# p2004dr/visual-slam

Measured on AMD Instinct MI355X. Metric: frames/sec (extract+match+pose) at 640×480, 2000 ORB, 1/2/4/8 MI355X, higher is better.
Workload: dtype u8

## Files before the change

visual-slam_amd/csrc/orb_kernels.hip:

```cpp
#include <cstring>

#include "common.h"
#include "select_replay.h"
#include "fast_score.h"

__constant__ __attribute__((aligned(16))) int8_t c_pattern[256 * 4] = {
#include "orb_pattern.inc"
};

#define WAVE 64

__device__ __forceinline__ int reflect101(int p, int len) {
    if (len == 1) return 0;
    while (p < 0 || p >= len) p = p < 0 ? -p : 2 * len - 2 - p;
    return p;
}

__device__ __forceinline__ void xcd_map(uint32_t lin, uint32_t per, uint32_t inv_per, uint32_t batch, int& frame, int& item) {
    const uint32_t b8 = batch & ~7u, cut = per * b8;
    const bool head = lin < cut;
    const uint32_t n = head ? lin >> 3 : lin - cut;
    const uint32_t q = inv_per ? __umulhi(n, inv_per) : n;
    item = (int)(n - q * per);
    frame = (int)(head ? (lin & 7u) + 8u * q : b8 + q);
// ... 66 lines not shown

#define RS_TW 64
#define RS_TH 64
#define RS_SRC_ROWS 136
#define RS_SRC_PITCH 144

__global__ __launch_bounds__(256) void k_resize(const uint8_t* __restrict__ src, size_t src_fstride, int spitch, int sw, int sh,
                                                uint8_t* __restrict__ dst, size_t dst_fstride, int dpitch, int dw, int dh,
                                                const int* __restrict__ xofs, const int* __restrict__ xc1,
                                                const int* __restrict__ yofs, const int* __restrict__ yc1,
                                                uint32_t inv_per, uint32_t inv_gx, int org) {
    __shared__ __attribute__((aligned(16))) uint8_t s_src[RS_SRC_ROWS * RS_SRC_PITCH];
    __shared__ int s_xo[RS_TW], s_xc[RS_TW], s_yo[RS_TH], s_yc[RS_TH];
    const int tid = threadIdx.x;
    int bx = blockIdx.x, by = blockIdx.y, bz = blockIdx.z;
    {
        int rem;
        xcd_map(bx + gridDim.x * (by + gridDim.y * bz), gridDim.x * gridDim.y, inv_per, gridDim.z, bz, rem);
        by = (int)(inv_gx ? __umulhi((uint32_t)rem, inv_gx) : (uint32_t)rem);
        bx = rem - by * (int)gridDim.x;
    }
    const int tx0 = org + bx * RS_TW, ty0 = org + by * RS_TH;
    const uint8_t* s = src + (size_t)bz * src_fstride;
    const int sx0 = xofs[tx0], sx1 = min(xofs[min(tx0 + RS_TW - 1, dw - 1)] + 1, sw - 1);
    const int sy0 = yofs[ty0], sy1 = min(yofs[min(ty0 + RS_TH - 1, dh - 1)] + 1, sh - 1);
    const int sxa = sx0 & ~3;
    const int ncols = sx1 - sxa + 1, nrows = sy1 - sy0 + 1;
    if (ncols > RS_SRC_PITCH || nrows > RS_SRC_ROWS) return;
    if (tid < RS_TW) {
        int x = min(tx0 + tid, dw - 1);
        s_xo[tid] = xofs[x];
        s_xc[tid] = xc1[x];
    } else if (tid < RS_TW + RS_TH) {
        int y = min(ty0 + tid - RS_TW, dh - 1);
        s_yo[tid - RS_TW] = yofs[y];
        s_yc[tid - RS_TW] = yc1[y];
    }
    if ((spitch & 3) == 0 && (((size_t)s) & 3) == 0) {
        const int ndw = (ncols + 3) >> 2;
        const uint32_t inv = 0x100000u / (uint32_t)ndw + 1u;
        const uint8_t* s0 = s + (size_t)sy0 * spitch + sxa;
        for (int i = tid; i < nrows * ndw; i += 256) {
            const uint32_t r = ((uint32_t)i * inv) >> 20, c4 = (uint32_t)i - r * (uint32_t)ndw;
            ((uint32_t*)(s_src + r * RS_SRC_PITCH))[c4] = *(const uint32_t*)(s0 + r * (uint32_t)spitch + 4u * c4);
        }
    } else {
        for (int i = tid; i < nrows * ncols; i += 256) {
            int r = i / ncols, cc = i - r * ncols;
            s_src[r * RS_SRC_PITCH + cc] = s[(size_t)(sy0 + r) * spitch + sxa + cc];
        }
    }
    __syncthreads();
    const int c0 = (tid & 15) * 4, x = tx0 + c0;
    if (x >= dw) return;
    int ox[4], ox1[4];
    uint32_t mx1[4];
#pragma unroll
    for (int k = 0; k < 4; k++) {
        ox[k] = s_xo[c0 + k] - sxa;
        ox1[k] = min(s_xo[c0 + k] + 1, sw - 1) - sxa;
        mx1[k] = s_xc[c0 + k];
    }
#pragma unroll
    for (int half = 0; half < RS_TH / 16; half++) {
        const int ry = (tid >> 4) + 16 * half, y = ty0 + ry;
        if (y >= dh) break;
        const int oy = s_yo[ry] - sy0, oy1 = min(s_yo[ry] + 1, sh - 1) - sy0;
        const uint32_t my1 = s_yc[ry], my0 = 256 - my1;
        const uint8_t* r0 = s_src + oy * RS_SRC_PITCH;
        const uint8_t* r1 = s_src + oy1 * RS_SRC_PITCH;
        uint32_t packed = 0;
#pragma unroll
        for (int k = 0; k < 4; k++) {
            const uint32_t mx0 = 256 - mx1[k];
            uint32_t h0 = mx0 * r0[ox[k]] + mx1[k] * r0[ox1[k]];
            uint32_t h1 = mx0 * r1[ox[k]] + mx1[k] * r1[ox1[k]];
            uint32_t v = my0 * h0 + my1 * h1;
            packed |= ((v + 32768u) >> 16) << (8 * k);
        }
        *(uint32_t*)(dst + (size_t)bz * dst_fstride + (size_t)y * dpitch + x) = packed;
    }
}


#define RS2_ROWS 136
#define RS2_UNR 5

__device__ __forceinline__ uint2 rs2_hrow(uint32_t w0, uint32_t w1, uint32_t w2, uint32_t sh8, const uint32_t (&sel)[4],
                                          const uint32_t (&coef)[4]) {
    const uint32_t u0 = __builtin_amdgcn_alignbyte(w1, w0, sh8), u1 = __builtin_amdgcn_alignbyte(w2, w1, sh8);
    uint32_t hv[4];
#pragma unroll
    for (int k = 0; k < 4; k++) hv[k] = udot2(__builtin_amdgcn_perm(u1, u0, sel[k]), coef[k], 0u);
    return make_uint2(hv[0] | (hv[1] << 16), hv[2] | (hv[3] << 16));
}

__device__ __forceinline__ uint32_t rs2_vrow(uint2 a, uint2 b, uint32_t e) {
    const uint32_t c1 = e >> 16, cy = (256u - c1) | (c1 << 16);
    const uint32_t v0 = udot2(__builtin_amdgcn_perm(b.x, a.x, 0x05040100u), cy, 32768u);
    const uint32_t v1 = udot2(__builtin_amdgcn_perm(b.x, a.x, 0x07060302u), cy, 32768u);
    const uint32_t v2 = udot2(__builtin_amdgcn_perm(b.y, a.y, 0x05040100u), cy, 32768u);
    const uint32_t v3 = udot2(__builtin_amdgcn_perm(b.y, a.y, 0x07060302u), cy, 32768u);
    return __builtin_amdgcn_perm(v1, v0, 0x0C0C0602u) | (__builtin_amdgcn_perm(v3, v2, 0x0C0C0602u) << 16);
}

__device__ __forceinline__ uint32_t hi16_pair_sat_u8(uint32_t a, uint32_t b) {
    uint32_t d;
    asm("v_sat_pk_u8_i16 %0, %1" : "=v"(d) : "v"(__builtin_amdgcn_perm(b, a, 0x07060302u)));
    return d;
}

__device__ __forceinline__ uint4 blur_row_quad(const uint32_t* pw0, const uint32_t* pw1, uint32_t g0, uint32_t g1, uint32_t g2,
                                               uint32_t g3) {
    const uint32_t ta = g0 | (g1 << 8) | (g2 << 16) | (g3 << 24), tb = g2 | (g1 << 8) | (g0 << 16);
    uint32_t o[2][4];
#pragma unroll
    for (int h = 0; h < 2; h++) {
        const uint32_t* pw = h ? pw1 : pw0;
        const uint32_t w0 = pw[0], w1 = pw[1], w2 = pw[2];
        o[h][0] = __builtin_amdgcn_udot4(__builtin_amdgcn_alignbyte(w1, w0, 1), ta, __builtin_amdgcn_udot4(__builtin_amdgcn_alignbyte(w2, w1, 1), tb, 0, false), false);
        o[h][1] = __builtin_amdgcn_udot4(__builtin_amdgcn_alignbyte(w1, w0, 2), ta, __builtin_amdgcn_udot4(__builtin_amdgcn_alignbyte(w2, w1, 2), tb, 0, false), false);
        o[h][2] = __builtin_amdgcn_udot4(__builtin_amdgcn_alignbyte(w1, w0, 3), ta, __builtin_amdgcn_udot4(__builtin_amdgcn_alignbyte(w2, w1, 3), tb, 0, false), false);
        o[h][3] = __builtin_amdgcn_udot4(w1, ta, __builtin_amdgcn_udot4(w2, tb, 0, false), false);
    }
    return make_uint4(o[0][0] | (o[1][0] << 16), o[0][1] | (o[1][1] << 16), o[0][2] | (o[1][2] << 16), o[0][3] | (o[1][3] << 16));
}

__device__ __forceinline__ void blur_col_quad(const uint32_t* sr, int pitch, uint32_t g0, uint32_t g1, uint32_t g2, uint32_t g3,
                                              uint32_t& pe, uint32_t& po) {
    const uint32_t e0 = g0 | (g1 << 16), e1 = g2 | (g3 << 16), e2 = g2 | (g1 << 16), e3 = g0;
    const uint32_t d0 = g0 << 16, d1 = g1 | (g2 << 16), d2 = g3 | (g2 << 16), d3 = g1 | (g0 << 16);
    uint4 v[4];
#pragma unroll
    for (int j = 0; j < 4; j++) v[j] = *(const uint4*)(sr + j * pitch);
    uint32_t se[4], so[4];
#pragma unroll
    for (int k = 0; k < 4; k++) {
        const uint32_t a0 = k == 0 ? v[0].x : k == 1 ? v[0].y : k == 2 ? v[0].z : v[0].w;
        const uint32_t a1 = k == 0 ? v[1].x : k == 1 ? v[1].y : k == 2 ? v[1].z : v[1].w;
        const uint32_t a2 = k == 0 ? v[2].x : k == 1 ? v[2].y : k == 2 ? v[2].z : v[2].w;
        const uint32_t a3 = k == 0 ? v[3].x : k == 1 ? v[3].y : k == 2 ? v[3].z : v[3].w;
        se[k] = udot2(a0, e0, udot2(a1, e1, udot2(a2, e2, udot2(a3, e3, 1u << 15))));
        so[k] = udot2(a0, d0, udot2(a1, d1, udot2(a2, d2, udot2(a3, d3, 1u << 15))));
    }
    pe = hi16_pair_sat_u8(se[0], se[1]) | (hi16_pair_sat_u8(se[2], se[3]) << 16);
    po = hi16_pair_sat_u8(so[0], so[1]) | (hi16_pair_sat_u8(so[2], so[3]) << 16);
}

#define RB_PW 80
#define RB_PH 80
#define RB_WR 88
#define RB_WP 96
#define RB_SR_BYTES ((RB_PH / 2 + 4) * RB_PW * 4)
struct BlurOut {
    uint8_t* dst;
    size_t fstride;
    int pitch, margin;
    uint32_t taps;
};

template <bool RS2_BLUR>
__global__ __launch_bounds__(256) void k_resize2(const uint8_t* __restrict__ src, size_t src_fstride, int spitch, int sw, int sh,
                                                 uint8_t* __restrict__ dst, size_t dst_fstride, int dpitch, int dw, int dh,
                                                 const uint32_t* __restrict__ xpk, const uint32_t* __restrict__ ypk,
                                                 uint32_t inv_per, uint32_t inv_gx, int org, BlurOut bo) {
    const int tid = threadIdx.x;
    if constexpr (RS2_BLUR) {
        __shared__ __attribute__((aligned(16))) uint8_t s_px[RB_WR * RB_WP];
        __shared__ __attribute__((aligned(16))) uint32_t s_row[RB_SR_BYTES / 4];
        int bx = blockIdx.x, by = blockIdx.y, bz = blockIdx.z;
        {
            int rem;
            xcd_map(bx + gridDim.x * (by + gridDim.y * bz), gridDim.x * gridDim.y, inv_per, gridDim.z, bz, rem);
            by = (int)(inv_gx ? __umulhi((uint32_t)rem, inv_gx) : (uint32_t)rem);
            bx = rem - by * (int)gridDim.x;
        }
        const int tx0 = org + bx * RS_TW, ty0 = org + by * RS_TH;
        const uint32_t ey0 = ypk[ty0], ey1 = ypk[ty0 + RS_TH - 1], ex1 = xpk[tx0 + RS_TW - 1];
        const int sy0 = (int)(ey0 & 0x7FFFu), sy1 = (int)(ey1 & 0x7FFFu) + (int)((ey1 >> 15) & 1u);
        const int ab0 = (int)(xpk[tx0] & 0x7FFCu), ax1 = (int)(ex1 & 0x7FFFu) + (int)((ex1 >> 15) & 1u) + 1;
        const int bm = bo.margin;
        const int r0 = by == 0 ? bm : sy0, r1 = by == (int)gridDim.y - 1 ? sh - bm : (int)(ypk[ty0 + RS_TH] & 0x7FFFu);
        const int c0 = bx == 0 ? bm : ab0, c1 = bx == (int)gridDim.x - 1 ? (sw - bm + 3) & ~3 : (int)(xpk[tx0 + RS_TW] & 0x7FFCu);
        const int wy0 = min(r0 - 3, sy0), wy1 = max(r1 + 3, sy1 + 1);
        const int wx0 = min(c0 - 4, ab0), wx1 = max(c1 + 4, (ax1 + 3) & ~3);
        const int nwr = wy1 - wy0, ndw = (wx1 - wx0) >> 2;
        const uint8_t* img = src + (size_t)bz * src_fstride;
        const int cg = tid & 15, rr = tid >> 4;
        const uint4 xe = *(const uint4*)(xpk + tx0 + 4 * cg);
        uint32_t ye[RS_TH / 16];
#pragma unroll
        for (int half = 0; half < RS_TH / 16; half++) ye[half] = ypk[ty0 + rr + 16 * half];
        {
            constexpr int TRIPS = (RB_WR * (RB_WP / 4 - 2) + 255) / 256;
            const uint32_t inv = 0x100000u / (uint32_t)ndw + 1u;
            const bool inside = wy0 >= 0 && wy1 <= sh && wx0 >= 0 && wx1 <= sw;
            uint32_t v[TRIPS];
#pragma unroll
            for (int t = 0; t < TRIPS; t++) {
                const int i = min(tid + 256 * t, nwr * ndw - 1);
                const uint32_t r = ((uint32_t)i * inv) >> 20, c4 = (uint32_t)i - r * (uint32_t)ndw;
                const int x0 = wx0 + 4 * (int)c4;
                if (inside) {
                    v[t] = *(const uint32_t*)(img + (uint32_t)((wy0 + (int)r) * spitch + x0));
                } else {
                    const uint8_t* row = img + (uint32_t)(reflect101(wy0 + (int)r, sh) * spitch);
                    if (x0 >= 0 && x0 + 3 < sw) v[t] = *(const uint32_t*)(row + x0);
                    else {
                        uint32_t u = 0;
#pragma unroll
                        for (int b = 0; b < 4; b++) u |= (uint32_t)row[reflect101(x0 + b, sw)] << (8 * b);
                        v[t] = u;
                    }
                }
            }
#pragma unroll
            for (int t = 0; t < TRIPS; t++) {
                const int i = tid + 256 * t;
                if (i < nwr * ndw) {
                    const uint32_t r = ((uint32_t)i * inv) >> 20, c4 = (uint32_t)i - r * (uint32_t)ndw;
                    ((uint32_t*)(s_px + r * RB_WP))[c4] = v[t];
                }
            }
        }
        __syncthreads();
        {
            const uint32_t xk[4] = {xe.x, xe.y, xe.z, xe.w};
            const int ox0 = (int)(xk[0] & 0x7FFFu), ab = ox0 & ~3;
            const uint32_t sh8 = (uint32_t)(ox0 & 3);
            uint32_t sel[4], coef[4];
#pragma unroll
            for (int k = 0; k < 4; k++) {
                const uint32_t a = (xk[k] & 0x7FFFu) - (uint32_t)ox0, b = a + ((xk[k] >> 15) & 1u), c1k = xk[k] >> 16;
                sel[k] = a | (b << 16) | 0x0C000C00u;
                coef[k] = (256u - c1k) | (c1k << 16);
            }
            const int x = tx0 + 4 * cg;
            const uint32_t* pw = (const uint32_t*)(s_px + (ab - wx0));
#pragma unroll
            for (int half = 0; half < RS_TH / 16; half++) {
                const int y = ty0 + rr + 16 * half;
                if (x >= dw || y >= dh) break;
                const uint32_t e = ye[half];
                const int oy = (int)(e & 0x7FFFu) - wy0, oy1 = oy + (int)((e >> 15) & 1u);
                const uint32_t* p0 = pw + oy * (RB_WP / 4);
                const uint32_t* p1 = pw + oy1 * (RB_WP / 4);
                const uint2 a = rs2_hrow(p0[0], p0[1], p0[2], sh8, sel, coef), b = rs2_hrow(p1[0], p1[1], p1[2], sh8, sel, coef);
                *(uint32_t*)(dst + (size_t)bz * dst_fstride + (size_t)y * dpitch + x) = rs2_vrow(a, b, e);
            }
        }
        const uint32_t g0 = bo.taps & 255u, g1 = (bo.taps >> 8) & 255u, g2 = (bo.taps >> 16) & 255u, g3 = bo.taps >> 24;
        const int nq = (c1 - c0) >> 2, npr = (r1 - r0 + 7) >> 1, nop = (r1 - r0 + 1) >> 1;
        const uint32_t invq = 0x100000u / (uint32_t)max(nq, 1) + 1u;
        {
            const uint8_t* base = s_px + (r0 - 3 - wy0) * RB_WP + (c0 - 4 - wx0);
            for (int t = tid; t < npr * nq; t += 256) {
                const int p = (int)(((uint32_t)t * invq) >> 20), q = t - p * nq;
                const uint32_t* pw = (const uint32_t*)(base + 2 * p * RB_WP + 4 * q);
                *(uint4*)(s_row + p * RB_PW + 4 * q) = blur_row_quad(pw, pw + RB_WP / 4, g0, g1, g2, g3);
            }
        }
        __syncthreads();
        {
            uint8_t* out0 = bo.dst + (size_t)bz * bo.fstride;
            for (int t = tid; t < nop * nq; t += 256) {
                const int p = (int)(((uint32_t)t * invq) >> 20), q = t - p * nq;
                uint32_t pe, po;
                blur_col_quad(s_row + p * RB_PW + 4 * q, RB_PW, g0, g1, g2, g3, pe, po);
                const int y = r0 + 2 * p;
                uint8_t* out = out0 + (size_t)y * bo.pitch + c0 + 4 * q;
                *(uint32_t*)out = pe;
                if (y + 1 < r1) *(uint32_t*)(out + bo.pitch) = po;
            }
        }
        return;
    }
    __shared__ __attribute__((aligned(16))) uint2 s_h[RS2_ROWS][16];
    int bx = blockIdx.x, by = blockIdx.y, bz = blockIdx.z;
    {
        int rem;
        xcd_map(bx + gridDim.x * (by + gridDim.y * bz), gridDim.x * gridDim.y, inv_per, gridDim.z, bz, rem);
        by = (int)(inv_gx ? __umulhi((uint32_t)rem, inv_gx) : (uint32_t)rem);
        bx = rem - by * (int)gridDim.x;
    }
    const int tx0 = org + bx * RS_TW, ty0 = org + by * RS_TH;
    const uint32_t ey0 = ypk[ty0], ey1 = ypk[min(ty0 + RS_TH - 1, dh - 1)];
    const int sy0 = (int)(ey0 & 0x7FFFu), sy1 = (int)(ey1 & 0x7FFFu) + (int)((ey1 >> 15) & 1u);
    const int nrows = sy1 - sy0 + 1;
    if (nrows > RS2_ROWS) return;
    const int cg = tid & 15, rr = tid >> 4;
    const uint4 xe = *(const uint4*)(xpk + tx0 + 4 * cg);
    uint32_t ye[RS_TH / 16];
#pragma unroll
    for (int half = 0; half < RS_TH / 16; half++) ye[half] = ypk[ty0 + rr + 16 * half];
    const uint32_t xk[4] = {xe.x, xe.y, xe.z, xe.w};
    const int ox0 = (int)(xk[0] & 0x7FFFu), ab = ox0 & ~3;
    const uint32_t sh8 = (uint32_t)(ox0 & 3);
    uint32_t sel[4], coef[4];
#pragma unroll
    for (int k = 0; k < 4; k++) {
        const uint32_t a = (xk[k] & 0x7FFFu) - (uint32_t)ox0, b = a + ((xk[k] >> 15) & 1u), c1 = xk[k] >> 16;
        sel[k] = a | (b << 16) | 0x0C000C00u;
        coef[k] = (256u - c1) | (c1 << 16);
    }
    const int o1 = min(ab + 4, spitch - 4), o2 = min(ab + 8, spitch - 4);
    const uint8_t* s0 = src + (size_t)bz * src_fstride + (size_t)sy0 * spitch;
    for (int r0 = rr; r0 < nrows; r0 += 16 * RS2_UNR) {
        uint32_t w[RS2_UNR][3];
#pragma unroll
        for (int i = 0; i < RS2_UNR; i++) {
            const uint8_t* row = s0 + (uint32_t)(min(r0 + 16 * i, nrows - 1) * spitch);
            w[i][0] = *(const uint32_t*)(row + ab); w[i][1] = *(const uint32_t*)(row + o1); w[i][2] = *(const uint32_t*)(row + o2);
        }
#pragma unroll
        for (int i = 0; i < RS2_UNR; i++) {
            const int r = r0 + 16 * i;
            if (r >= nrows) break;
            s_h[r][cg] = rs2_hrow(w[i][0], w[i][1], w[i][2], sh8, sel, coef);
        }
    }
    __syncthreads();
    const int x = tx0 + 4 * cg;
    if (x >= dw) return;
#pragma unroll
    for (int half = 0; half < RS_TH / 16; half++) {
        const int y = ty0 + rr + 16 * half;
        if (y >= dh) break;
        const uint32_t e = ye[half];
        const int oy = (int)(e & 0x7FFFu) - sy0, oy1 = oy + (int)((e >> 15) & 1u);
        const uint32_t packed = rs2_vrow(s_h[oy][cg], s_h[oy1][cg], e);
        *(uint32_t*)(dst + (size_t)bz * dst_fstride + (size_t)y * dpitch + x) = packed;
    }
}

static int resize_org(const LevelInfo& d, int margin) { return (d.w > 2 * margin + 8 && d.h > 2 * margin + 8) ? margin : 0; }

bool orb_plan_resize_blur(const Plan& P, int L, const uint32_t* xp, size_t nx, const uint32_t* yp, size_t ny, int margin, int blur_margin) {
    const LevelInfo& s = P.lv[L - 1];
    const LevelInfo& d = P.lv[L];
    const int bm = blur_margin, org = resize_org(d, margin);
    if (bm < 0 || (bm & 3)) return false;
    const int gx = (d.w - 2 * org + RS_TW - 1) / RS_TW, gy = (d.h - 2 * org + RS_TH - 1) / RS_TH;
    if (gx < 1 || gy < 1 || (size_t)(org + gx * RS_TW + 1) > nx || (size_t)(org + gy * RS_TH + 1) > ny) return false;
    for (int by = 0; by < gy; by++) {
        const int ty0 = org + by * RS_TH;
        const uint32_t ey1 = yp[ty0 + RS_TH - 1];
        const int sy0 = (int)(yp[ty0] & 0x7FFFu), sy1 = (int)(ey1 & 0x7FFFu) + (int)((ey1 >> 15) & 1u);
        const int r0 = by == 0 ? bm : sy0, r1 = by == gy - 1 ? s.h - bm : (int)(yp[ty0 + RS_TH] & 0x7FFFu);
        const int wy0 = std::min(r0 - 3, sy0), wy1 = std::max(r1 + 3, sy1 + 1);
// ... 612 lines not shown
                }
            }
        }
    }
    __syncthreads();
    const int N1 = a_lds ? replay::wg_retain_best<NT, uint32_t>(s_A, N, 2 * lv.quota, P.select_order, a_rpos, a_bl, tid, &s_ws)
                         : replay::wg_retain_best<NT, uint32_t>(gA, N, 2 * lv.quota, P.select_order, g_rpos, g_bl, tid, &s_ws);
    const size_t b_off = a_lds ? (((size_t)N1 * 4 + 15) & ~(size_t)15) : 0;
    const bool b_lds = b_off + sel_need_bytes(N1, 8) <= (size_t)buf_bytes;
    uint64_t* s_B = (uint64_t*)(s_buf + b_off);
    uint16_t* b_rpos = (uint16_t*)((uint8_t*)s_B + (size_t)N1 * 8);
    unsigned long long* b_bl = (unsigned long long*)((uint8_t*)b_rpos + ((((size_t)N1 / 2 + 1) * 2 + 7) & ~(size_t)7));
    const uint8_t* img = level_ptr(P, L, gray, pyr, frame);
    FinalKp* fin = fin_all + (size_t)frame * P.fin_stride + lv.fin_off;
    if (a_lds && b_lds) select_harris<NT>(P, lv, img, s_A, s_B, N1, b_rpos, b_bl, fin, fin_cnt_out, flags, &s_ws, s_hw, L);
    else if (a_lds) select_harris<NT>(P, lv, img, s_A, gB, N1, g_rpos, g_bl, fin, fin_cnt_out, flags, &s_ws, s_hw, L);
    else if (b_lds) select_harris<NT>(P, lv, img, gA, s_B, N1, b_rpos, b_bl, fin, fin_cnt_out, flags, &s_ws, s_hw, L);
    else select_harris<NT>(P, lv, img, gA, gB, N1, g_rpos, g_bl, fin, fin_cnt_out, flags, &s_ws, s_hw, L);
}

int orb_launch_select(mo_ctx* c, const uint8_t* d_gray, int batch, int level_lo, int level_hi) {
    const Plan& P = c->plan;
    level_lo = std::max(level_lo, 0); level_hi = std::min(level_hi, P.nlevels);
    if (level_lo >= level_hi) return MO_OK;
    const size_t pref_bytes = (((size_t)c->pb.max_strips + 1) * sizeof(int) + 15) & ~(size_t)15;
    const size_t attr_bytes = SEL_BUF_BYTES + ((((size_t)SEL_MAXSTRIPS + 1) * sizeof(int) + 15) & ~(size_t)15);
    int rc;
    if ((rc = mo_raise_dyn_lds(c, (const void*)k_select<SEL_THREADS>, (int)attr_bytes)) ||
        (rc = mo_raise_dyn_lds(c, (const void*)k_select<SEL_THREADS_LATENCY>, (int)attr_bytes)))
        return rc;
    const dim3 grid(batch, level_hi - level_lo);
    if (batch <= 2)
        hipLaunchKernelGGL(k_select<SEL_THREADS_LATENCY>, grid, dim3(SEL_THREADS_LATENCY), SEL_BUF_BYTES + pref_bytes, c->stream, P, d_gray, c->pb.d_pyr, c->pb.d_cand,
                           c->pb.d_strip_cnt, c->pb.d_scratch, c->pb.scratch_stride, c->pb.d_fin, c->pb.d_fin_cnt, c->flags_cur, level_lo, SEL_BUF_BYTES, c->pb.d_dtodo);
    else
        hipLaunchKernelGGL(k_select<SEL_THREADS>, grid, dim3(SEL_THREADS), SEL_BUF_BYTES + pref_bytes, c->stream, P, d_gray, c->pb.d_pyr, c->pb.d_cand,
                           c->pb.d_strip_cnt, c->pb.d_scratch, c->pb.scratch_stride, c->pb.d_fin, c->pb.d_fin_cnt, c->flags_cur, level_lo, SEL_BUF_BYTES, c->pb.d_dtodo);
    HIPCHK(c, hipGetLastError());
    return MO_OK;
}

__global__ __launch_bounds__(SEL_THREADS) void k_retain_probe(const float* resp, int n, int n_points, int order, uint64_t* rec,
                                                              uint16_t* rpos, unsigned long long* bl, int32_t* out, int* nout) {
    __shared__ replay::WgScratch<SEL_THREADS> s_ws;
    for (int i = threadIdx.x; i < n; i += SEL_THREADS) rec[i] = ((uint64_t)__float_as_uint(resp[i]) << 32) | (uint32_t)i;
    __syncthreads();
    int keep = replay::wg_retain_best<SEL_THREADS, uint64_t>(rec, n, n_points, order, rpos, bl, threadIdx.x, &s_ws);
    __syncthreads();
    for (int i = threadIdx.x; i < keep; i += SEL_THREADS) out[i] = (int32_t)(rec[i] & 0xFFFFFFFFu);
    if (threadIdx.x == 0) *nout = keep;
}

int orb_launch_retain_probe(mo_ctx* c, const float* d_resp, int n, int n_points, int order, int32_t* d_order, int* d_nout) {
    size_t nn = (size_t)std::max(n, 1);
    size_t rec_b = nn * sizeof(uint64_t), rpos_b = ((nn / 2 + 4) * 2 + 7) & ~(size_t)7, bl_b = (nn / 64 + 8) * 8;
    int rc = c->d_tmp.reserve_exact(c, rec_b + rpos_b + bl_b);
    if (rc) return rc;
    uint8_t* b = c->d_tmp;
    hipLaunchKernelGGL(k_retain_probe, dim3(1), dim3(SEL_THREADS), 0, c->stream, d_resp, n, n_points, order, (uint64_t*)b,
                       (uint16_t*)(b + rec_b), (unsigned long long*)(b + rec_b + rpos_b), d_order, d_nout);
    HIPCHK(c, hipGetLastError());
    return MO_OK;
}

__device__ __forceinline__ float fast_atan2_deg(float y, float x) {
    const float p1 = 0.9997878412794807f * (float)(180 / 3.14159265358979323846);
    const float p3 = -0.3258083974640975f * (float)(180 / 3.14159265358979323846);
    const float p5 = 0.1555786518463281f * (float)(180 / 3.14159265358979323846);
    const float p7 = -0.04432655554792128f * (float)(180 / 3.14159265358979323846);
    float ax = fabsf(x), ay = fabsf(y);
    float a, c, c2;
    if (ax >= ay) {
        c = ay / (ax + (float)2.2204460492503131e-16);
        c2 = c * c;
        a = (((p7 * c2 + p5) * c2 + p3) * c2 + p1) * c;
    } else {
        c = ax / (ay + (float)2.2204460492503131e-16);
        c2 = c * c;
        a = 90.f - (((p7 * c2 + p5) * c2 + p3) * c2 + p1) * c;
    }
    if (x < 0) a = 180.f - a;
    if (y < 0) a = 360.f - a;
    return a;
}

__device__ __forceinline__ int wave_sum(int v) {
#pragma unroll
    for (int o = 32; o > 0; o >>= 1) v += __shfl_xor(v, o, 64);
    return v;
}

template <bool BOUNDS>
__device__ __forceinline__ void rbrief_wave(const uint8_t* blur, int bpitch, const uint8_t* raw, int rpitch, int lw, int lh,
                                            int cx, int cy, float angle_deg, uint8_t* desc, int lane) {
    float angle = angle_deg;
    angle *= (float)(3.14159265358979323846 / 180.f);
    double sd, cd;
    sincos((double)angle, &sd, &cd);
    float a = (float)cd, b = (float)sd;
    unsigned nib = 0;
#pragma unroll
    for (int k = 0; k < 4; k++) {
        const int8_t* pt = &c_pattern[(lane * 4 + k) * 4];
        float fx0 = (float)pt[0], fy0 = (float)pt[1], fx1 = (float)pt[2], fy1 = (float)pt[3];
        int ix0 = __float2int_rn(fx0 * a - fy0 * b), iy0 = __float2int_rn(fx0 * b + fy0 * a);
        int ix1 = __float2int_rn(fx1 * a - fy1 * b), iy1 = __float2int_rn(fx1 * b + fy1 * a);
        int x0 = cx + ix0, y0 = cy + iy0, x1 = cx + ix1, y1 = cy + iy1;
        int t0, t1;
        if (BOUNDS) {
            t0 = (x0 >= 0 && x0 < lw && y0 >= 0 && y0 < lh) ? blur[(size_t)y0 * bpitch + x0]
                                                           : raw[(size_t)reflect101(y0, lh) * rpitch + reflect101(x0, lw)];
            t1 = (x1 >= 0 && x1 < lw && y1 >= 0 && y1 < lh) ? blur[(size_t)y1 * bpitch + x1]
                                                           : raw[(size_t)reflect101(y1, lh) * rpitch + reflect101(x1, lw)];
        } else {
            t0 = blur[(size_t)y0 * bpitch + x0];
            t1 = blur[(size_t)y1 * bpitch + x1];
        }
        nib |= (t0 < t1 ? 1u : 0u) << k;
    }
    unsigned hi = __shfl_down(nib, 1, 64);
    if ((lane & 1) == 0) desc[lane >> 1] = (uint8_t)(nib | (hi << 4));
}

#define DG 16

__device__ __forceinline__ int group_sum(int v) {
#pragma unroll
    for (int o = DG / 2; o > 0; o >>= 1) v += __shfl_xor(v, o, 64);
    return v;
}

typedef const __attribute__((address_space(3))) uint8_t lds_cu8;
__device__ __forceinline__ uint16_t rbrief_u16_lds(uint32_t lds_base, int ppitch, float a, float b, const float4* pat, int gl) {
    const uint32_t base = lds_base - 0x4B400000u - 0x400000u * (uint32_t)ppitch;
    uint32_t val = 0;
#ifndef RB_UNROLL
#define RB_UNROLL 16
#endif
#pragma unroll 1
    for (int k0 = 16 - RB_UNROLL; k0 >= 0; k0 -= RB_UNROLL) {
#pragma unroll
        for (int kk = RB_UNROLL - 1; kk >= 0; kk--) {
            const float4 pt = pat[(k0 + kk) * DG + gl];
            const int jx0 = __float_as_int((pt.x * a - pt.y * b) + 12582912.f), jy0 = __float_as_int((pt.x * b + pt.y * a) + 12582912.f);
            const int jx1 = __float_as_int((pt.z * a - pt.w * b) + 12582912.f), jy1 = __float_as_int((pt.z * b + pt.w * a) + 12582912.f);
            const uint32_t a0 = (uint32_t)__mul24(jy0, ppitch) + (base + (uint32_t)jx0), a1 = (uint32_t)__mul24(jy1, ppitch) + (base + (uint32_t)jx1);
            const int t0 = *(lds_cu8*)(uintptr_t)a0, t1 = *(lds_cu8*)(uintptr_t)a1;
            val = __builtin_amdgcn_alignbit(val, (uint32_t)(t0 - t1), 31);
        }
    }
    return (uint16_t)val;
}

#define DT_RAW_P ((DT_W + 30 + 7 + 7) & ~7)
#define DT_RAW_ROWS (DT_H + 30)
#define DT_BLR_P ((DT_W + 38 + 7 + 7) & ~7)
#define DT_BLR_ROWS (DT_H + 38)
#ifndef DT_NT
#define DT_NT 256
#endif
#ifdef DT_WAVES
#define DT_WAVES_ATTR __attribute__((amdgpu_waves_per_eu(DT_WAVES, 8)))
#else
#define DT_WAVES_ATTR
#endif
#define DT_CHUNK 512
#define DT_LIST (DT_NT > 160 ? DT_NT : 160)
#define DT_RAW_LD ((DT_RAW_ROWS * (DT_RAW_P / 8) + DT_NT - 1) / DT_NT)
#define DT_BLR_LD ((DT_BLR_ROWS * (DT_BLR_P / 8) + DT_NT - 1) / DT_NT)

template <int NROWS, int NQ, int NLD>
__device__ __forceinline__ void tile_issue(const uint8_t* img, int pitch, int h, int ry0, int cx_al, int tid, uint2 (&v)[NLD]) {
    const int last_q = (pitch >> 3) - 1;
#pragma unroll
    for (int u = 0; u < NLD; u++) {
        const int t = min(tid + u * DT_NT, NROWS * NQ - 1), r = t / NQ, c = t - r * NQ;
        const int y = min(max(ry0 + r, 0), h - 1), q = min(max((cx_al >> 3) + c, 0), last_q);
        v[u] = ((const uint2*)(img + (size_t)y * pitch))[q];
    }
}
template <int NROWS, int NQ, int NLD>
__device__ __forceinline__ void tile_store(uint8_t* lds, int tid, const uint2 (&v)[NLD]) {
#pragma unroll
    for (int u = 0; u < NLD; u++) {
        const int t = tid + u * DT_NT, r = t / NQ, c = t - r * NQ;
        if (t < NROWS * NQ) *(uint2*)(lds + r * (NQ * 8) + 8 * c) = v[u];
    }
}
__device__ __forceinline__ void tile_load_bytes(const uint8_t* img, int pitch, int w, int h, int ry0, int nrows, int cx0, int lp, uint8_t* lds, int tid) {
    for (int i = tid; i < nrows * lp; i += DT_NT) {
        const int r = i / lp, c = i - r * lp;
        const int y = min(max(ry0 + r, 0), h - 1), x = min(max(cx0 + c, 0), w - 1);
        lds[i] = img[(size_t)y * pitch + x];
    }
}

template <bool HAS_DESC, bool RARE>
__device__ __forceinline__ void describe_tile(const Plan& P, int frame, int tile, int tiles_per_frame, int split, int nsplit ,
                                              const uint32_t* __restrict__ tile_tab,
                                              const uint8_t* __restrict__ gray, const uint8_t* __restrict__ pyr,
                                              const uint8_t* __restrict__ blur, const FinalKp* __restrict__ fin_all,
                                              const int* __restrict__ fin_cnt, mo_keypoint* __restrict__ kps,
                                              uint8_t* __restrict__ desc, int cap, int* __restrict__ counts, int* flags,
                                              const uint32_t* __restrict__ icw, int* __restrict__ todo) {
    __shared__ __attribute__((aligned(16))) uint8_t s_tile[HAS_DESC ? DT_BLR_ROWS * DT_BLR_P : DT_RAW_ROWS * DT_RAW_P];
    __shared__ __attribute__((aligned(16))) float4 s_pat[HAS_DESC ? 256 : 1];
    __shared__ uint32_t s_list[DT_LIST];
    __shared__ float2 s_ab[DT_LIST];
    __shared__ int s_n;
    static_assert(DT_BLR_ROWS * DT_BLR_P >= DT_RAW_ROWS * DT_RAW_P, "the blurred tile is the larger one");
    const uint32_t te = tile_tab[tile];
    const int L = te & 0xFF;
    const int x0 = P.lv[L].bx0 + (int)((te >> 8) & 0xFFF) * DT_W, y0 = P.lv[L].by0 + (int)(te >> 20) * DT_H;
    const int lpitch = P.lv[L].pitch, lbpitch = P.lv[L].bpitch, lw = P.lv[L].w, lh = P.lv[L].h;
    const float lscale = P.lv[L].scale;
    const int tid = threadIdx.x, grp = tid / DG, gl = tid % DG;
    const int* fc = fin_cnt + (size_t)frame * MO_MAX_LEVELS;
    int total = 0, base = 0, nL = 0;
    {
        int cn[MO_MAX_LEVELS];
#pragma unroll
        for (int l = 0; l < MO_MAX_LEVELS; l++) cn[l] = fc[l];
#pragma unroll
        for (int l = 0; l < MO_MAX_LEVELS; l++) {
            const int n = l < P.nlevels ? cn[l] : 0;
            if (l == L) { base = total; nL = n; }
            total += n;
        }
    }
    if (!RARE && tile == 0 && split == 0 && tid == 0) {
        counts[frame] = total;
        if (total > cap) atomicOr(&flags[0], 2);
    }
    nL = min(nL, max(cap - base, 0));
    if (nL == 0) return;
    const uint8_t* img = level_ptr(P, L, gray, pyr, frame);
    const uint8_t* bl = blur + (size_t)frame * P.blur_stride + P.lv[L].boff;
    const bool al_raw = (lpitch & 7) == 0 && (((size_t)img) & 7) == 0;
    const bool al_blr = (((size_t)bl) & 7) == 0;
    const int xr_al = al_raw ? (x0 - 15) & ~7 : x0 - 15, lead_r = (x0 - 15) - xr_al;
    const int xb_al = al_blr ? (x0 - 19) & ~7 : x0 - 19;
    const FinalKp* fin = fin_all + (size_t)frame * P.fin_stride + P.lv[L].fin_off;
    FinalKp fk[DT_CHUNK / DT_NT];
    uint2 vr[DT_RAW_LD], vb[DT_BLR_LD];
    if (!RARE) {
#pragma unroll
        for (int u = 0; u < DT_CHUNK / DT_NT; u++) fk[u] = fin[min(tid + u * DT_NT, nL - 1)];
        if (al_raw) tile_issue<DT_RAW_ROWS, DT_RAW_P / 8, DT_RAW_LD>(img, lpitch, lh, y0 - 15, xr_al, tid, vr);
    }
    uint32_t wt[8], mk[8];
    {
        const uint4* w = (const uint4*)(icw + gl * 16);
        const uint4 w0 = w[0], w1 = w[1], k0 = w[2], k1 = w[3];
        wt[0] = w0.x; wt[1] = w0.y; wt[2] = w0.z; wt[3] = w0.w; wt[4] = w1.x; wt[5] = w1.y; wt[6] = w1.z; wt[7] = w1.w;
        mk[0] = k0.x; mk[1] = k0.y; mk[2] = k0.z; mk[3] = k0.w; mk[4] = k1.x; mk[5] = k1.y; mk[6] = k1.z; mk[7] = k1.w;
    }
    if (HAS_DESC && tid < 256 && DT_NT >= 256) {
        const int l = tid & 15, k = tid >> 4;
        const int8_t* pt = &c_pattern[(l * 16 + k) * 4];
        s_pat[k * DG + l] = make_float4((float)pt[0], (float)pt[1], (float)pt[2], (float)pt[3]);
    } else if (HAS_DESC && DT_NT < 256) {
        for (int i = tid; i < 256; i += DT_NT) {
            const int l = i & 15, k = i >> 4;
            const int8_t* pt = &c_pattern[(l * 16 + k) * 4];
            s_pat[k * DG + l] = make_float4((float)pt[0], (float)pt[1], (float)pt[2], (float)pt[3]);
        }
    }
    const int row_b_w = gl == 15 ? 0 : 1;
    const uint32_t tile_lds = (uint32_t)(uintptr_t)s_tile;

    auto select = [&](int c0, int sub) {
#pragma unroll
        for (int u = 0; u < DT_CHUNK / DT_NT; u++) {
            const int i = c0 + tid + u * DT_NT;
            const int dx = (int)fk[u].x - x0, dy = (int)fk[u].y - y0;
            if ((sub < 0 || u == sub) && i < nL && (unsigned)dx < DT_W && (unsigned)dy < DT_H && (i & (nsplit - 1)) == split) {
                const int pos = atomicAdd(&s_n, 1);
                if (pos < DT_LIST) {
                    s_list[pos] = (uint32_t)(i - c0) | ((uint32_t)dx << 9) | ((uint32_t)dy << 17);
                    s_ab[pos].y = fk[u].response;
                }
            }
        }
    };
    auto phase_a = [&](int c0, int n) {
        for (int j = grp; j < n; j += DT_NT / DG) {
            const uint32_t e = s_list[j];
            const int i = c0 + (int)(e & 0x1FF), dx = (int)((e >> 9) & 255), dy = (int)(e >> 17);
            const int k = base + i, x = x0 + dx, y = y0 + dy;
            const int col = dx + lead_r, offr = col & 3;
            int m10 = 0, m01 = 0;
#pragma unroll
            for (int rr = 0; rr < 2; rr++) {
                const int row_i = rr == 0 ? gl : 30 - gl;
                const uint32_t* rowp = (const uint32_t*)(s_tile + (dy + row_i) * DT_RAW_P + (col & ~3));
                uint32_t pxw[9];
#pragma unroll
                for (int c4 = 0; c4 < 9; c4++) pxw[c4] = rowp[c4];
                uint32_t sw = 0, rs = 0;
#pragma unroll
                for (int c4 = 0; c4 < 8; c4++) {
                    const uint32_t a = __builtin_amdgcn_alignbyte(pxw[c4 + 1], pxw[c4], (uint32_t)offr);
                    sw = __builtin_amdgcn_udot4(a, wt[c4], sw, false);
                    rs = __builtin_amdgcn_udot4(a, mk[c4], rs, false);
                }
                const int wgt = rr == 0 ? 1 : row_b_w;
                m10 += wgt * ((int)sw - 16 * (int)rs);
                m01 += wgt * (row_i - 15) * (int)rs;
            }
            m10 = group_sum(m10);
            m01 = group_sum(m01);
            const float angle = fast_atan2_deg((float)m01, (float)m10);
            if (gl == 0) {
                mo_keypoint* o = kps + (size_t)frame * cap + k;
                o->x = (float)x * lscale; o->y = (float)y * lscale;
                o->size = 31 * lscale;
                o->angle = angle;
                o->response = s_ab[j].y;
                o->octave = L;
                o->class_id = -1;
                s_ab[j].x = angle;
            }
        }
    };
    auto phase_b = [&](int n) {
        for (int j = tid; j < n; j += DT_NT) {
            float angle = s_ab[j].x;
            angle *= (float)(3.14159265358979323846 / 180.f);
            double sd, cd;
            sincos((double)angle, &sd, &cd);
            s_ab[j] = make_float2((float)cd, (float)sd);
        }
    };
    auto phase_c = [&](int c0, int n) {
        for (int j = grp; j < n; j += DT_NT / DG) {
            const uint32_t ex = s_list[j];
            const int i = c0 + (int)(ex & 0x1FF), dx = (int)((ex >> 9) & 255), dy = (int)(ex >> 17);
            const int k = base + i;
            const float px = (float)(x0 + dx) * lscale, py = (float)(y0 + dy) * lscale, inv = 1.f / lscale;
            const int cx = __float2int_rn(px * inv), cy = __float2int_rn(py * inv);
            const float2 ab = s_ab[j];
            int glo = gl;
            asm volatile("" : "+v"(glo));
            *(uint16_t*)(desc + ((size_t)frame * cap + k) * 32 + 2 * gl) =
                rbrief_u16_lds(tile_lds + (uint32_t)((cy - (y0 - 19)) * DT_BLR_P + (cx - xb_al)), DT_BLR_P, ab.x, ab.y, s_pat, glo);
        }
    };

    if (!RARE) {
        if (tid == 0) s_n = 0;
        if (al_raw) tile_store<DT_RAW_ROWS, DT_RAW_P / 8, DT_RAW_LD>(s_tile, tid, vr);
        else tile_load_bytes(img, lpitch, lw, lh, y0 - 15, DT_RAW_ROWS, xr_al, DT_RAW_P, s_tile, tid);
        __syncthreads();
        select(0, -1);
        __syncthreads();
        const int n0 = s_n;
        if (nL > DT_CHUNK || n0 > DT_LIST) {
            if (tid == 0 && (split == 0 || n0 > DT_LIST)) todo[1 + atomicAdd(&todo[0], 1)] = frame * tiles_per_frame + tile;
            return;
        }
        phase_a(0, n0);
        if (HAS_DESC) {
            if (al_blr) tile_issue<DT_BLR_ROWS, DT_BLR_P / 8, DT_BLR_LD>(bl, lbpitch, lh, y0 - 19, xb_al, tid, vb);
            __syncthreads();
            phase_b(n0);
            if (al_blr) tile_store<DT_BLR_ROWS, DT_BLR_P / 8, DT_BLR_LD>(s_tile, tid, vb);
            else tile_load_bytes(bl, lbpitch, lw, lh, y0 - 19, DT_BLR_ROWS, xb_al, DT_BLR_P, s_tile, tid);
            __syncthreads();
            phase_c(0, n0);
        }
        return;
    }
    for (int c0 = 0; c0 < nL; c0 += DT_CHUNK) {
#pragma unroll
        for (int u = 0; u < DT_CHUNK / DT_NT; u++) fk[u] = fin[min(c0 + tid + u * DT_NT, nL - 1)];
#pragma unroll 1
        for (int sub = 0; sub < DT_CHUNK / DT_NT; sub++) {
            __syncthreads();
            if (tid == 0) s_n = 0;
            tile_load_bytes(img, lpitch, lw, lh, y0 - 15, DT_RAW_ROWS, xr_al, DT_RAW_P, s_tile, tid);
            __syncthreads();
            select(c0, sub);
            __syncthreads();
            const int n = s_n;
            phase_a(c0, n);
            if (HAS_DESC) {
                __syncthreads();
                tile_load_bytes(bl, lbpitch, lw, lh, y0 - 19, DT_BLR_ROWS, xb_al, DT_BLR_P, s_tile, tid);
                phase_b(n);
                __syncthreads();
                phase_c(c0, n);
            }
        }
    }
    __syncthreads();
}

template <bool HAS_DESC>
__global__ __launch_bounds__(DT_NT) DT_WAVES_ATTR void k_describe_tiles(Plan P, const uint32_t* __restrict__ tile_tab, uint32_t inv_per,
                                                          const uint8_t* __restrict__ gray, const uint8_t* __restrict__ pyr,
                                                          const uint8_t* __restrict__ blur, const FinalKp* __restrict__ fin_all,
                                                          const int* __restrict__ fin_cnt, mo_keypoint* __restrict__ kps,
                                                          uint8_t* __restrict__ desc, int cap, int* __restrict__ counts, int* flags,
                                                          const uint32_t* __restrict__ icw, int* __restrict__ todo) {
    int frame = blockIdx.y, tile = blockIdx.x;
    xcd_map(blockIdx.x + gridDim.x * blockIdx.y, gridDim.x, inv_per, gridDim.y, frame, tile);
    describe_tile<HAS_DESC, false>(P, frame, tile, (int)gridDim.x, (int)blockIdx.z, (int)gridDim.z, tile_tab, gray, pyr, blur, fin_all, fin_cnt, kps, desc, cap, counts, flags, icw, todo);
}

template <bool HAS_DESC>
__global__ __launch_bounds__(DT_NT) void k_describe_tiles_rare(Plan P, const uint32_t* __restrict__ tile_tab, int tiles_per_frame,
                                                               const uint8_t* __restrict__ gray, const uint8_t* __restrict__ pyr,
                                                               const uint8_t* __restrict__ blur, const FinalKp* __restrict__ fin_all,
                                                               const int* __restrict__ fin_cnt, mo_keypoint* __restrict__ kps,
                                                               uint8_t* __restrict__ desc, int cap, int* __restrict__ counts, int* flags,
                                                               const uint32_t* __restrict__ icw, int* __restrict__ todo) {
    const int n = todo[0];
    for (int e = blockIdx.x; e < n; e += gridDim.x) {
        const int ft = todo[1 + e];
        describe_tile<HAS_DESC, true>(P, ft / tiles_per_frame, ft % tiles_per_frame, tiles_per_frame, 0, 1, tile_tab, gray, pyr, blur, fin_all, fin_cnt, kps,
                                      desc, cap, counts, flags, icw, todo);
    }
}

int orb_launch_describe(mo_ctx* c, const uint8_t* d_gray, int batch, mo_keypoint* d_kps, uint8_t* d_desc, int cap, int* d_counts) {
    const Plan& P = c->plan;
    if (c->pb.n_dtiles == 0) {
        HIPCHK(c, hipMemsetAsync(d_counts, 0, (size_t)batch * sizeof(int), c->stream));
        return MO_OK;
    }
    const dim3 grid(c->pb.n_dtiles, batch, batch <= 2 ? DT_SPLIT_LATENCY : 1);
    const uint32_t inv_per = grid.x > 1 ? 0xFFFFFFFFu / grid.x + 1u : 0u;
    const uint32_t* const dtile_tab = c->pb.d_tables + c->pb.dtile_tab;
    const uint32_t* icw = c->pb.d_tables + c->pb.dtile_icw;
    const dim3 rare_grid(std::min(c->pb.n_dtiles * batch, 256));
    if (d_desc) {
        hipLaunchKernelGGL(k_describe_tiles<true>, grid, dim3(DT_NT), 0, c->stream, P, dtile_tab, inv_per, d_gray, c->pb.d_pyr, c->pb.d_blur,
                           c->pb.d_fin, c->pb.d_fin_cnt, d_kps, d_desc, cap, d_counts, c->flags_cur, icw, c->pb.d_dtodo);
        hipLaunchKernelGGL(k_describe_tiles_rare<true>, rare_grid, dim3(DT_NT), 0, c->stream, P, dtile_tab, c->pb.n_dtiles, d_gray, c->pb.d_pyr,
                           c->pb.d_blur, c->pb.d_fin, c->pb.d_fin_cnt, d_kps, d_desc, cap, d_counts, c->flags_cur, icw, c->pb.d_dtodo);
    } else {
        hipLaunchKernelGGL(k_describe_tiles<false>, grid, dim3(DT_NT), 0, c->stream, P, dtile_tab, inv_per, d_gray, c->pb.d_pyr, c->pb.d_blur,
                           c->pb.d_fin, c->pb.d_fin_cnt, d_kps, d_desc, cap, d_counts, c->flags_cur, icw, c->pb.d_dtodo);
        hipLaunchKernelGGL(k_describe_tiles_rare<false>, rare_grid, dim3(DT_NT), 0, c->stream, P, dtile_tab, c->pb.n_dtiles, d_gray, c->pb.d_pyr,
                           c->pb.d_blur, c->pb.d_fin, c->pb.d_fin_cnt, d_kps, d_desc, cap, d_counts, c->flags_cur, icw, c->pb.d_dtodo);
    }
    HIPCHK(c, hipGetLastError());
    return MO_OK;
}

#define DC_TILE_BYTES 13312
#define DC_MAXREC 256
__global__ __launch_bounds__(256) void k_describe_cells(Plan P, const uint8_t* __restrict__ blur, const mo_keypoint* __restrict__ kps,
                                                        const int32_t* __restrict__ kbase, uint8_t* __restrict__ desc, int cap, int cw,
                                                        int ch, int tpitch) {
    __shared__ __attribute__((aligned(16))) uint8_t s_tile[DC_TILE_BYTES];
    __shared__ __attribute__((aligned(16))) float4 s_pat[256];
    __shared__ float2 s_ab[DC_MAXREC];
    __shared__ uint32_t s_ctr[DC_MAXREC];
    const int cell = blockIdx.x, frame = blockIdx.y, tid = threadIdx.x, grp = tid / DG, gl = tid % DG;
    const int i0 = kbase[(size_t)frame * 65 + cell], n = min(kbase[(size_t)frame * 65 + cell + 1] - i0, DC_MAXREC);
    if (n <= 0) return;
    const int x0 = (cell & 7) * cw, y0 = (cell >> 3) * ch;
    const LevelInfo lv = P.lv[0];
    const uint8_t* bl = blur + (size_t)frame * P.blur_stride + lv.boff;
    const int xb_al = (x0 - 19) & ~7, rows = ch + 38, nq = tpitch >> 3, last_q = (lv.bpitch >> 3) - 1;
    {
        constexpr int U = 8;
        const int total = rows * nq;
        const uint32_t inv = 0xFFFFFFFFu / (uint32_t)nq + 1u;
        for (int t0 = tid; t0 < total; t0 += 256 * U) {
            uint2 v[U];
#pragma unroll
            for (int u = 0; u < U; u++) {
                const int t = min(t0 + u * 256, total - 1), r = (int)__umulhi((uint32_t)t, inv), c = t - r * nq;
                const int y = min(max(y0 - 19 + r, 0), lv.h - 1), q = min(max((xb_al >> 3) + c, 0), last_q);
                v[u] = ((const uint2*)(bl + (size_t)y * lv.bpitch))[q];
            }
#pragma unroll
            for (int u = 0; u < U; u++) {
                const int t = t0 + u * 256, r = (int)__umulhi((uint32_t)t, inv), c = t - r * nq;
                if (t < total) *(uint2*)(s_tile + r * tpitch + 8 * c) = v[u];
            }
        }
    }
    {
        const int l = tid & 15, k = tid >> 4;
        const int8_t* pt = &c_pattern[(l * 16 + k) * 4];
        s_pat[k * DG + l] = make_float4((float)pt[0], (float)pt[1], (float)pt[2], (float)pt[3]);
    }
    const uint32_t tile_lds = (uint32_t)(uintptr_t)s_tile;
    for (int j = tid; j < n; j += 256) {
        const mo_keypoint kp = kps[(size_t)frame * cap + i0 + j];
        const float inv = 1.f / lv.scale;
        const int cx = __float2int_rn(kp.x * inv), cy = __float2int_rn(kp.y * inv);
        float angle = kp.angle;
        angle *= (float)(3.14159265358979323846 / 180.f);
        double sd, cd;
        sincos((double)angle, &sd, &cd);
        s_ab[j] = make_float2((float)cd, (float)sd);
        s_ctr[j] = tile_lds + (uint32_t)((cy - (y0 - 19)) * tpitch + (cx - xb_al));
    }
    __syncthreads();
    for (int j = grp; j < n; j += 256 / DG) {
        const float2 ab = s_ab[j];
        int glo = gl;
        asm volatile("" : "+v"(glo));
        *(uint16_t*)(desc + ((size_t)frame * cap + i0 + j) * 32 + 2 * gl) = rbrief_u16_lds(s_ctr[j], tpitch, ab.x, ab.y, s_pat, glo);
    }
}

int orb_launch_describe_cells(mo_ctx* c, const mo_keypoint* d_kps, const int32_t* d_kbase, uint8_t* d_desc, int cap, int batch) {
    const Plan& P = c->plan;
    const int cw = P.w / 8, ch = P.h / 8;
    const int tpitch = (cw + 38 + 7 + 7) & ~7;
    if ((size_t)tpitch * (ch + 38) > DC_TILE_BYTES || P.edge_threshold < 19) return MO_ERR_UNSUPPORTED;
    hipLaunchKernelGGL(k_describe_cells, dim3(64, batch), dim3(256), 0, c->stream, P, c->pb.d_blur, d_kps, d_kbase, d_desc, cap, cw, ch, tpitch);
    HIPCHK(c, hipGetLastError());
    return MO_OK;
}

__global__ __launch_bounds__(256) void k_describe_given(Plan P, const uint8_t* __restrict__ gray,
                                                        const uint8_t* __restrict__ pyr, const uint8_t* __restrict__ blur,
                                                        const mo_keypoint* __restrict__ kps, int n, const int* __restrict__ n_dev,
                                                        int n_stride, uint8_t* __restrict__ desc) {
// ... 25 lines not shown
```

Measured before the change: 118,900.

## Stage image tiles into LDS with 16-byte loads and shared staging registers

```diff
diff --git a/visual-slam_amd/csrc/orb_kernels.hip b/visual-slam_amd/csrc/orb_kernels.hip
--- a/visual-slam_amd/csrc/orb_kernels.hip
+++ b/visual-slam_amd/csrc/orb_kernels.hip
@@ -242,6 +242,7 @@
 #define RB_WR 88
 #define RB_WP 96
 #define RB_SR_BYTES ((RB_PH / 2 + 4) * RB_PW * 4)
+struct __attribute__((packed, aligned(4))) Dwords4 { uint32_t x, y, z, w; };
 struct BlurOut {
     uint8_t* dst;
     size_t fstride;
@@ -281,10 +282,25 @@
         uint32_t ye[RS_TH / 16];
 #pragma unroll
         for (int half = 0; half < RS_TH / 16; half++) ye[half] = ypk[ty0 + rr + 16 * half];
-        {
+        const bool inside = wy0 >= 0 && wy1 <= sh && wx0 >= 0 && wx1 <= sw;
+        const int np16 = (ndw + 3) >> 2;
+        if (inside && wx0 + 16 * np16 <= spitch) {
+            constexpr int TRIPS = (RB_WR + 31) / 32;
+            static_assert(RB_WP % 16 == 0 && RB_WP / 16 <= 8, "a window row is at most 8 pieces of 16 bytes");
+            const int p = tid & 7, r = tid >> 3;
+            const int rows_left = p < np16 ? nwr - r : 0;
+            const uint32_t goff = (uint32_t)((wy0 + r) * spitch + wx0 + 16 * p);
+            uint8_t* const lrow = s_px + r * RB_WP + 16 * p;
+            Dwords4 v[TRIPS];
+#pragma unroll
+            for (int t = 0; t < TRIPS; t++)
+                if (32 * t < rows_left) v[t] = *(const Dwords4*)(img + (size_t)(32 * t) * (uint32_t)spitch + goff);
+#pragma unroll
+            for (int t = 0; t < TRIPS; t++)
+                if (32 * t < rows_left) *(uint4*)(lrow + 32 * t * RB_WP) = make_uint4(v[t].x, v[t].y, v[t].z, v[t].w);
+        } else {
             constexpr int TRIPS = (RB_WR * (RB_WP / 4 - 2) + 255) / 256;
             const uint32_t inv = 0x100000u / (uint32_t)ndw + 1u;
-            const bool inside = wy0 >= 0 && wy1 <= sh && wx0 >= 0 && wx1 <= sw;
             uint32_t v[TRIPS];
 #pragma unroll
             for (int t = 0; t < TRIPS; t++) {
@@ -1203,10 +1219,13 @@
     return (uint16_t)val;
 }
 
-#define DT_RAW_P ((DT_W + 30 + 7 + 7) & ~7)
+#define DT_RAW_P ((DT_W + 30 + 15 + 15) & ~15)
 #define DT_RAW_ROWS (DT_H + 30)
-#define DT_BLR_P ((DT_W + 38 + 7 + 7) & ~7)
+#define DT_BLR_P ((DT_W + 38 + 15 + 15) & ~15)
 #define DT_BLR_ROWS (DT_H + 38)
+#define DT_RAW_NQ ((DT_W + 30 + 7 + 7) >> 3)
+#define DT_BLR_NQ ((DT_W + 38 + 7 + 7) >> 3)
+static_assert(((DT_RAW_P / 4) & 1) || ((DT_RAW_P / 4) & 7) == 4, "raw tile pitch: odd, or an odd multiple of 4 dwords");
 #ifndef DT_NT
 #define DT_NT 256
 #endif
@@ -1217,26 +1236,58 @@
 #endif
 #define DT_CHUNK 512
 #define DT_LIST (DT_NT > 160 ? DT_NT : 160)
-#define DT_RAW_LD ((DT_RAW_ROWS * (DT_RAW_P / 8) + DT_NT - 1) / DT_NT)
-#define DT_BLR_LD ((DT_BLR_ROWS * (DT_BLR_P / 8) + DT_NT - 1) / DT_NT)
+#define DT_RAW_LD ((DT_RAW_ROWS * DT_RAW_NQ + DT_NT - 1) / DT_NT)
+#define DT_BLR_LD ((DT_BLR_ROWS * DT_BLR_NQ + DT_NT - 1) / DT_NT)
+#define DT_RAW_NP (DT_RAW_P / 16)
+#define DT_BLR_NP (DT_BLR_P / 16)
+#define DT_RAW_LD16 ((DT_RAW_ROWS + DT_NT / DT_RAW_NP - 1) / (DT_NT / DT_RAW_NP))
+#define DT_BLR_LD16 ((DT_BLR_ROWS + DT_NT / DT_BLR_NP - 1) / (DT_NT / DT_BLR_NP))
+#define DT_MAX2(a, b) ((a) > (b) ? (a) : (b))
+#define DT_STAGE_REGS DT_MAX2(DT_MAX2(2 * DT_RAW_LD, 2 * DT_BLR_LD), DT_MAX2(4 * DT_RAW_LD16, 4 * DT_BLR_LD16))
 
 template <int NROWS, int NQ, int NLD>
-__device__ __forceinline__ void tile_issue(const uint8_t* img, int pitch, int h, int ry0, int cx_al, int tid, uint2 (&v)[NLD]) {
+__device__ __forceinline__ void tile_issue(const uint8_t* img, int pitch, int h, int ry0, int cx_al, int tid, uint32_t (&v)[DT_STAGE_REGS]) {
     const int last_q = (pitch >> 3) - 1;
 #pragma unroll
     for (int u = 0; u < NLD; u++) {
         const int t = min(tid + u * DT_NT, NROWS * NQ - 1), r = t / NQ, c = t - r * NQ;
         const int y = min(max(ry0 + r, 0), h - 1), q = min(max((cx_al >> 3) + c, 0), last_q);
-        v[u] = ((const uint2*)(img + (size_t)y * pitch))[q];
-    }
-}
-template <int NROWS, int NQ, int NLD>
-__device__ __forceinline__ void tile_store(uint8_t* lds, int tid, const uint2 (&v)[NLD]) {
+        const uint2 d = ((const uint2*)(img + (size_t)y * pitch))[q];
+        v[2 * u] = d.x; v[2 * u + 1] = d.y;
+    }
+}
+template <int NROWS, int NQ, int LP, int NLD>
+__device__ __forceinline__ void tile_store(uint8_t* lds, int tid, const uint32_t (&v)[DT_STAGE_REGS]) {
 #pragma unroll
     for (int u = 0; u < NLD; u++) {
         const int t = tid + u * DT_NT, r = t / NQ, c = t - r * NQ;
-        if (t < NROWS * NQ) *(uint2*)(lds + r * (NQ * 8) + 8 * c) = v[u];
-    }
+        if (t < NROWS * NQ) *(uint2*)(lds + r * LP + 8 * c) = make_uint2(v[2 * u], v[2 * u + 1]);
+    }
+}
+typedef uint32_t dt_u32x4 __attribute__((ext_vector_type(4)));
+template <int NP>
+__device__ __forceinline__ void tile_lane16(int pitch, int ry0, int cx_al, int nrows, int ncols, int tid, uint32_t& goff, uint32_t& loff, int& rows_left,
+                                            uint32_t& last) {
+    const int g = tid / NP, l = tid - g * NP;
+    const bool on = g < DT_NT / NP && 16 * l < ncols && g < nrows;
+    rows_left = on ? nrows - g : 0;
+    goff = (uint32_t)(ry0 * pitch + cx_al) + (on ? (uint32_t)(g * pitch + 16 * l) : 0u);
+    loff = (uint32_t)(g * (NP * 16) + 16 * l);
+    last = on ? (uint32_t)((rows_left - 1) / (DT_NT / NP) * (DT_NT / NP) * pitch) : 0u;
+}
+template <int NP, int NLD>
+__device__ __forceinline__ void tile_issue16(const uint8_t* img, int pitch, uint32_t goff, uint32_t last, uint32_t (&v)[DT_STAGE_REGS]) {
+#pragma unroll
+    for (int u = 0; u < NLD; u++) {
+        const dt_u32x4 d = *(const dt_u32x4*)(img + (goff + min((uint32_t)(u * (DT_NT / NP) * pitch), last)));
+        v[4 * u] = d.x; v[4 * u + 1] = d.y; v[4 * u + 2] = d.z; v[4 * u + 3] = d.w;
+    }
+}
+template <int NP, int NLD>
+__device__ __forceinline__ void tile_store16(uint8_t* lds, uint32_t loff, int rows_left, const uint32_t (&v)[DT_STAGE_REGS]) {
+#pragma unroll
+    for (int u = 0; u < NLD; u++)
+        if (u * (DT_NT / NP) < rows_left) *(dt_u32x4*)(lds + loff + u * (DT_NT / NP) * (NP * 16)) = dt_u32x4{v[4 * u], v[4 * u + 1], v[4 * u + 2], v[4 * u + 3]};
 }
 __device__ __forceinline__ void tile_load_bytes(const uint8_t* img, int pitch, int w, int h, int ry0, int nrows, int cx0, int lp, uint8_t* lds, int tid) {
     for (int i = tid; i < nrows * lp; i += DT_NT) {
@@ -1289,23 +1340,35 @@
     const uint8_t* bl = blur + (size_t)frame * P.blur_stride + P.lv[L].boff;
     const bool al_raw = (lpitch & 7) == 0 && (((size_t)img) & 7) == 0;
     const bool al_blr = (((size_t)bl) & 7) == 0;
-    const int xr_al = al_raw ? (x0 - 15) & ~7 : x0 - 15, lead_r = (x0 - 15) - xr_al;
-    const int xb_al = al_blr ? (x0 - 19) & ~7 : x0 - 19;
+    const int nkc = min(DT_W, P.lv[L].bx0 + P.lv[L].bw - x0), nkr = min(DT_H, P.lv[L].by0 + P.lv[L].bh - y0);
+    const int lead_r16 = (x0 - 15) & 15, lead_b16 = (x0 - 19) & 15;
+    const int ncols_r = lead_r16 + nkc + 30, ncols_b = lead_b16 + nkc + 38;
+    const bool w16_raw = !RARE && ((lpitch | (int)(size_t)img) & 15) == 0 && y0 - 15 >= 0 && y0 + nkr + 15 <= lh && x0 - 15 - lead_r16 >= 0 &&
+                         x0 - 15 - lead_r16 + ((ncols_r + 15) & ~15) <= lpitch;
+    const bool w16_blr = !RARE && ((lbpitch | (int)(size_t)bl) & 15) == 0 && y0 - 19 >= 0 && y0 + nkr + 19 <= lh && x0 - 19 - lead_b16 >= 0 &&
+                         x0 - 19 - lead_b16 + ((ncols_b + 15) & ~15) <= lbpitch;
+    const int xr_al = w16_raw ? x0 - 15 - lead_r16 : al_raw ? (x0 - 15) & ~7 : x0 - 15, lead_r = (x0 - 15) - xr_al;
+    const int xb_al = w16_blr ? x0 - 19 - lead_b16 : al_blr ? (x0 - 19) & ~7 : x0 - 19;
     const FinalKp* fin = fin_all + (size_t)frame * P.fin_stride + P.lv[L].fin_off;
     FinalKp fk[DT_CHUNK / DT_NT];
-    uint2 vr[DT_RAW_LD], vb[DT_BLR_LD];
+    uint32_t vs[DT_STAGE_REGS];
+    uint32_t goff = 0, loff = 0, last = 0;
+    int rows_left = 0;
     if (!RARE) {
 #pragma unroll
         for (int u = 0; u < DT_CHUNK / DT_NT; u++) fk[u] = fin[min(tid + u * DT_NT, nL - 1)];
-        if (al_raw) tile_issue<DT_RAW_ROWS, DT_RAW_P / 8, DT_RAW_LD>(img, lpitch, lh, y0 - 15, xr_al, tid, vr);
+        if (w16_raw) {
+            tile_lane16<DT_RAW_NP>(lpitch, y0 - 15, xr_al, nkr + 30, ncols_r, tid, goff, loff, rows_left, last);
+            tile_issue16<DT_RAW_NP, DT_RAW_LD16>(img, lpitch, goff, last, vs);
+        } else if (al_raw) tile_issue<DT_RAW_ROWS, DT_RAW_NQ, DT_RAW_LD>(img, lpitch, lh, y0 - 15, xr_al, tid, vs);
     }
     uint32_t wt[8], mk[8];
-    {
+    auto load_icw = [&]() {
         const uint4* w = (const uint4*)(icw + gl * 16);
         const uint4 w0 = w[0], w1 = w[1], k0 = w[2], k1 = w[3];
         wt[0] = w0.x; wt[1] = w0.y; wt[2] = w0.z; wt[3] = w0.w; wt[4] = w1.x; wt[5] = w1.y; wt[6] = w1.z; wt[7] = w1.w;
         mk[0] = k0.x; mk[1] = k0.y; mk[2] = k0.z; mk[3] = k0.w; mk[4] = k1.x; mk[5] = k1.y; mk[6] = k1.z; mk[7] = k1.w;
-    }
+    };
     if (HAS_DESC && tid < 256 && DT_NT >= 256) {
         const int l = tid & 15, k = tid >> 4;
         const int8_t* pt = &c_pattern[(l * 16 + k) * 4];
@@ -1400,8 +1463,10 @@
 
     if (!RARE) {
         if (tid == 0) s_n = 0;
-        if (al_raw) tile_store<DT_RAW_ROWS, DT_RAW_P / 8, DT_RAW_LD>(s_tile, tid, vr);
+        if (w16_raw) tile_store16<DT_RAW_NP, DT_RAW_LD16>(s_tile, loff, rows_left, vs);
+        else if (al_raw) tile_store<DT_RAW_ROWS, DT_RAW_NQ, DT_RAW_P, DT_RAW_LD>(s_tile, tid, vs);
         else tile_load_bytes(img, lpitch, lw, lh, y0 - 15, DT_RAW_ROWS, xr_al, DT_RAW_P, s_tile, tid);
+        load_icw();
         __syncthreads();
         select(0, -1);
         __syncthreads();
@@ -1412,16 +1477,21 @@
         }
         phase_a(0, n0);
         if (HAS_DESC) {
-            if (al_blr) tile_issue<DT_BLR_ROWS, DT_BLR_P / 8, DT_BLR_LD>(bl, lbpitch, lh, y0 - 19, xb_al, tid, vb);
+            if (w16_blr) {
+                tile_lane16<DT_BLR_NP>(lbpitch, y0 - 19, xb_al, nkr + 38, ncols_b, tid, goff, loff, rows_left, last);
+                tile_issue16<DT_BLR_NP, DT_BLR_LD16>(bl, lbpitch, goff, last, vs);
+            } else if (al_blr) tile_issue<DT_BLR_ROWS, DT_BLR_NQ, DT_BLR_LD>(bl, lbpitch, lh, y0 - 19, xb_al, tid, vs);
             __syncthreads();
             phase_b(n0);
-            if (al_blr) tile_store<DT_BLR_ROWS, DT_BLR_P / 8, DT_BLR_LD>(s_tile, tid, vb);
+            if (w16_blr) tile_store16<DT_BLR_NP, DT_BLR_LD16>(s_tile, loff, rows_left, vs);
+            else if (al_blr) tile_store<DT_BLR_ROWS, DT_BLR_NQ, DT_BLR_P, DT_BLR_LD>(s_tile, tid, vs);
             else tile_load_bytes(bl, lbpitch, lw, lh, y0 - 19, DT_BLR_ROWS, xb_al, DT_BLR_P, s_tile, tid);
             __syncthreads();
             phase_c(0, n0);
         }
         return;
     }
+    load_icw();
     for (int c0 = 0; c0 < nL; c0 += DT_CHUNK) {
 #pragma unroll
         for (int u = 0; u < DT_CHUNK / DT_NT; u++) fk[u] = fin[min(c0 + tid + u * DT_NT, nL - 1)];
```

Measured after the change: 121,100, median of 6. 1.02x the previous value.
